# FireMines/zk_stark_project

Measured on NVIDIA B200. Metric: stark_proofs_per_sec, higher is better.
Workload: dtype u128 mod p (f128 field, 4x u32 limbs), u32 BLAKE3

## Files before the change

### zk_stark_project_b200/csrc/kernels.cuh

```cuda
#pragma once
#include "f128.cuh"
#include "blake3.cuh"
#include "coin.cuh"

namespace zkb {

struct PowTab {
    const fe* lo;
    const fe* hi;
    uint32_t l1;
};
__device__ __forceinline__ fe powtab(const PowTab& t, uint32_t e) {
    fe a = fe_ldg(t.lo + (e & ((1u << t.l1) - 1u)));
    fe b = fe_ldg(t.hi + (e >> t.l1));
    return fe_mul(a, b);
}

struct LdeMat {
    fe* data;
    uint32_t log_n, log_beta, w, log_p;
    uint32_t log_shard, bw, bw_magic, view, q_self;
    uint64_t blk_stride;
    uint32_t k0, log_kc;
};
// ... 14 lines not shown
    const uint32_t panel = (uint32_t)(gid >> lslots);
    const uint32_t slot = m.view == 0 ? s : ((m.q_self << m.log_p) + s);
    const uint32_t k = m.k0 + (panel >> lt), t_low = panel & ((1u << lt) - 1u);
    const uint32_t i = t_low + (slot << lt);
    return {k, i, compact ? (((uint64_t)i << m.log_kc) + (k - m.k0)) : (((uint64_t)i << m.log_beta) + k - leaf0)};
}
__device__ __forceinline__ size_t lde_col_off(const LdeMat& m, uint32_t j) {
    const uint32_t blk = (j * m.bw_magic) >> 16;
    return (size_t)blk * m.blk_stride + ((size_t)(j - blk * m.bw) << m.log_p);
}
__device__ __forceinline__ size_t lde_addr(const LdeMat& m, uint32_t k, uint32_t i, uint32_t j) {
    return lde_row_base(m, k, i) + lde_col_off(m, j);
}

__global__ void k_transpose_cols(const fe* __restrict__ in, fe* __restrict__ out, uint32_t n, uint32_t wc, uint32_t out_stride) {
    __shared__ uint4 tile[32][33];
    const uint32_t i0 = blockIdx.x * 32, j0 = blockIdx.y * 32;
    for (uint32_t jj = threadIdx.y; jj < 32; jj += blockDim.y) {
        uint32_t j = j0 + jj, i = i0 + threadIdx.x;
        if (j < wc && i < n) {
            const fe v = fe_canon(fe_load(in + (size_t)j * n + i), 0);
            tile[jj][threadIdx.x] = make_uint4(v.x[0], v.x[1], v.x[2], v.x[3]);
        }
    }
    __syncthreads();
    for (uint32_t ii = threadIdx.y; ii < 32; ii += blockDim.y) {
        uint32_t i = i0 + ii, j = j0 + threadIdx.x;
        if (j < wc && i < n) reinterpret_cast<uint4*>(out)[(size_t)i * out_stride + j] = tile[threadIdx.x][ii];
    }
}

struct NttPass {
    const fe* in;
    fe* out;
    uint32_t log_n, a, b;
    uint32_t w_in, w_out;
    uint32_t col0_in, col0_out, ncols, cj;
    uint32_t n_cosets, coset0;
    uint64_t in_coset_stride, out_coset_stride;
    uint32_t coset;
    uint32_t inverse;
    uint32_t log_tab;
    uint32_t log_lde;
    uint32_t out_panel;
    uint32_t log_shard;
    uint32_t panel_k0, log_kc;
    uint32_t do_scale;
    fe scale;
    PowTab roots;
    const fe* pow3;
    const fe* tw_tab;
    uint32_t tw_four;
    uint32_t tile0;
};

__device__ __forceinline__ uint32_t bitrev(uint32_t v, uint32_t bits) { return bits == 0 ? 0u : (__brev(v) >> (32 - bits)); }

__device__ __forceinline__ fe tw_mul(const fe& x, const fe& w) { return fe_mul(x, w); }
__device__ __forceinline__ fe tw_mul(const fe& x, const fe4& w) { return fe_mul_pre4(x, w); }

template <int RHO, int NC, class TW>
__device__ __forceinline__ void ntt_unit(fe* __restrict__ col, const uint32_t rs, const uint32_t cstride, const TW* __restrict__ tw,
                                         const uint32_t base, const uint32_t lam0) {
    constexpr int R = 1 << RHO;
    fe x[NC][R];
    const uint32_t step = rs << lam0;
    fe* p = col + base * rs;
#pragma unroll
    for (int c = 0; c < NC; c++)
#pragma unroll
        for (int d = 0; d < R; d++) x[c][d] = p[d * step + c * cstride];
    const uint32_t base_low = base & ((1u << lam0) - 1u);
#pragma unroll
    for (int s = 0; s < RHO; s++) {
        const TW* twl = tw + ((1u << (lam0 + s)) - 1u) + base_low;
#pragma unroll
        for (int t = 0; t < (1 << s); t++) {
            const TW w = twl[(uint32_t)t << lam0];
#pragma unroll
            for (int g = 0; g < (R >> (s + 1)); g++) {
                const int d0 = g * (2 << s) + t, d1 = d0 + (1 << s);
#pragma unroll
                for (int c = 0; c < NC; c++) {
                    const fe u = x[c][d0];
                    const fe v = tw_mul(x[c][d1], w);
                    x[c][d0] = fe_add(u, v);
                    x[c][d1] = fe_sub(u, v);
                }
            }
        }
    }
#pragma unroll
    for (int c = 0; c < NC; c++)
#pragma unroll
        for (int d = 0; d < R; d++) p[d * step + c * cstride] = x[c][d];
}

__device__ __forceinline__ fe ntt_twiddle(const NttPass& p, uint32_t k, uint32_t t_low, uint32_t q) {
    const uint32_t logS = p.b - p.a;
    const uint32_t tab_mask = (1u << p.log_tab) - 1u;
    const uint32_t lam = 32 - __clz(q + 1);
    const uint32_t th = q + 1 - (1u << (lam - 1));
    const uint32_t l = p.a + lam;
    (void)logS;
    uint32_t e = (t_low << (p.log_tab - l)) + (th << (p.log_tab - lam));
    if (p.coset) e += (k << (p.log_n - l)) << (p.log_tab - p.log_lde);
// ... 73 lines not shown
        asm volatile("cp.async.commit_group;" ::: "memory");
    } else {
        const fe* t = p.tw_tab ? p.tw_tab + ((size_t)(k << p.a) + t_low) * (S - 1u) : nullptr;
        for (uint32_t q = threadIdx.x; q + 1 < S; q += blockDim.x) {
            const fe w = t ? fe_ldg(t + q) : ntt_twiddle(p, k, t_low, q);
            if (PRE) tw[q] = fe4_from(w); else tw1[q] = w;
        }
    }
    const uint32_t c_base = ct << log_cj;
    const uint32_t log_bd = 31 - __clz(blockDim.x), log_dv = log_bd - log_cj;
    const uint32_t jj_t = threadIdx.x & (cj - 1u), v_t = threadIdx.x >> log_cj, dv = 1u << log_dv;
    const uint32_t nrow = v_t < S ? ((S - 1u - v_t) >> log_dv) + 1u : 0u;
    const bool col_ok = c_base + jj_t < p.ncols;
    {
        const size_t vstride = ((size_t)p.w_in << (p.log_n - p.b)) << p.a;
        const fe* src = p.in + (size_t)kk * p.in_coset_stride + (((size_t)u0 << p.a) + t_low) * p.w_in + p.col0_in + c_base + jj_t +
                        (size_t)v_t * vstride;
        const size_t dstride = (size_t)dv * vstride;
        char* smc = reinterpret_cast<char*>(sm + jj_t);
        const uint32_t brs = (32u - logS) & 31u;
        const uint32_t rs16 = rs * 16u;
        uint32_t vs = v_t << brs;
        const uint32_t dvs = dv << brs;
        if (col_ok) {
#pragma unroll 4
            for (uint32_t i = 0; i < nrow; i++, vs += dvs, src += dstride) *reinterpret_cast<fe*>(smc + __brev(vs) * rs16) = fe_load(src);
        } else {
            for (uint32_t i = 0; i < nrow; i++, vs += dvs) *reinterpret_cast<fe*>(smc + __brev(vs) * rs16) = fe_zero();
        }
    }
    if (PRE) asm volatile("cp.async.wait_all;" ::: "memory");
    __syncthreads();
    if (PRE) { if (cj >= 16) ntt_rounds<2>(sm, tw, rs, log_cj, logS); else ntt_rounds<1>(sm, tw, rs, log_cj, logS); }
    else ntt_rounds<1>(sm, tw1, rs, log_cj, logS);
    if (p.out_panel) {
        const size_t panel = ((size_t)(k - p.panel_k0) << p.a) + t_low;
        const uint32_t lp = logS - p.log_shard;
        const size_t np = (size_t)1 << (p.log_kc + p.a);
        const size_t chunk_stride = (np * p.w_out) << lp;
        const bool wide = S >= blockDim.x;
        const uint32_t th0 = wide ? threadIdx.x : (threadIdx.x & (S - 1u)), dth = wide ? blockDim.x : S;
        const uint32_t jj0 = wide ? 0u : (threadIdx.x >> logS), log_djj = wide ? 0u : log_bd - logS, djj = 1u << log_djj;
        const uint32_t jend = min(cj, p.ncols - c_base);
        const uint32_t ncol = jj0 < jend ? ((jend - 1u - jj0) >> log_djj) + 1u : 0u;
        const size_t cstep = (size_t)djj << lp;
        fe* colp = p.out + ((panel * p.w_out + p.col0_out + c_base + jj0) << lp);
#pragma unroll 1
        for (uint32_t th = th0; th < S; th += dth) {
            fe* d = colp + (size_t)(th >> lp) * chunk_stride + (th & ((1u << lp) - 1u));
            const fe* s = sm + th * rs + jj0;
#pragma unroll 4
            for (uint32_t j = 0; j < ncol; j++, d += cstep, s += djj) fe_store(d, *s);
        }
    } else {
        const size_t tstride = (size_t)p.w_out << p.a;
        fe* dst = p.out + (size_t)kk * p.out_coset_stride + (((size_t)u0 << p.b) + t_low) * p.w_out + p.col0_out + c_base + jj_t +
                  (size_t)v_t * tstride;
        const size_t dstride = (size_t)dv * tstride;
        const fe* s = sm + v_t * rs + jj_t;
        const uint32_t sstep = dv * rs;
        if (col_ok) {
            if (p.do_scale) {
                for (uint32_t i = 0; i < nrow; i++, dst += dstride, s += sstep) fe_store(dst, fe_mul(*s, p.scale));
            } else {
#pragma unroll 4
                for (uint32_t i = 0; i < nrow; i++, dst += dstride, s += sstep) fe_store(dst, *s);
            }
        }
    }
}

__global__ void k_scale_pow(fe* x, uint64_t n, PowTab base, fe scale, uint64_t keep, uint32_t* __restrict__ bad_degree) {
    uint64_t m = (uint64_t)blockIdx.x * blockDim.x + threadIdx.x;
    if (m >= n) return;
    const fe v = fe_load(x + m);
    if (m >= keep) { if (!fe_is_zero(v)) atomicOr(bad_degree, 1u); return; }
    fe f = fe_mul(powtab(base, (uint32_t)m), scale);
    fe_store(x + m, fe_mul(v, f));
}

__global__ void __launch_bounds__(128) k_hash_lde_rows(const LdeMat m, uint32_t* __restrict__ leaves, uint64_t leaf0, uint32_t compact) {
    const uint64_t gid = (uint64_t)blockIdx.x * blockDim.x + threadIdx.x;
    const uint32_t lpf = lde_full_log_p(m), lt = m.log_n - lpf;
    const uint32_t log_rows = m.log_kc + lt + (m.view == 0 ? lpf : m.log_p);
    if (gid >> log_rows) return;
    const LdeLeaf L = lde_leaf(m, gid, leaf0, compact);
    uint32_t d[8];
    b3_hash_elems(m.data + lde_row_base(m, L.k, L.i), (size_t)1 << m.log_p, m.w, d, m.bw, m.bw_magic, m.blk_stride);
    uint4* o = reinterpret_cast<uint4*>(leaves + L.r * 8);
    o[0] = make_uint4(d[0], d[1], d[2], d[3]);
    o[1] = make_uint4(d[4], d[5], d[6], d[7]);
}
__global__ void __launch_bounds__(128) k_hash_lde_rows_split(const LdeMat m, uint32_t* __restrict__ leaves, uint64_t leaf0, uint32_t compact) {
    const uint64_t t = (uint64_t)blockIdx.x * blockDim.x + threadIdx.x;
    const uint32_t c = (uint32_t)t & 3u;
    const uint32_t lpf = lde_full_log_p(m), lt = m.log_n - lpf;
    const uint32_t log_rows = m.log_kc + lt + (m.view == 0 ? lpf : m.log_p);
    const bool live = ((t >> 2) >> log_rows) == 0;
    const LdeLeaf L = lde_leaf(m, live ? (t >> 2) : 0, leaf0, compact);
    const uint32_t nchunks = (m.w + 63u) / 64u;
    uint32_t cv[8], nb[8];
    if (c < nchunks) b3_chunk_cv_elems(m.data + lde_row_base(m, L.k, L.i), (size_t)1 << m.log_p, m.w, c, cv, m.bw, m.bw_magic, m.blk_stride);
    else {
#pragma unroll
        for (int q = 0; q < 8; q++) cv[q] = 0;
    }
// ... 287 lines not shown
    fe s = fe_zero();
    if (j < w) for (uint32_t c = gy; c < nchunks; c += 32) s = fe_add(s, fe_load(part + (size_t)c * w + j));
    red[gy][jx] = make_uint4(s.x[0], s.x[1], s.x[2], s.x[3]);
    __syncthreads();
    for (uint32_t h = 16; h > 0; h >>= 1) {
        if (gy < h) {
            uint4 o = red[gy + h][jx];
            fe t; t.x[0] = o.x; t.x[1] = o.y; t.x[2] = o.z; t.x[3] = o.w;
            s = fe_add(s, t);
            red[gy][jx] = make_uint4(s.x[0], s.x[1], s.x[2], s.x[3]);
        }
        __syncthreads();
    }
    if (gy == 0 && j < w) fe_store(out + j, s);
}
__global__ void __launch_bounds__(256) k_poly_eval_partial(const fe* __restrict__ coef, uint32_t n, uint32_t Q, const DevTs* __restrict__ ts,
                                                           fe* __restrict__ part) {
    const fe z = ts->z, zQ = ts->zR;
    const uint32_t t = blockIdx.x * blockDim.x + threadIdx.x;
    const uint32_t nt = (n + Q - 1) / Q;
    if (t >= nt) return;
    const fe* c = coef + (size_t)blockIdx.y * n;
    const uint32_t m0 = t * Q, m1 = min(n, m0 + Q);
    fe a = fe_zero();
    for (uint32_t m = m1; m-- > m0;) a = fe_add(fe_mul(a, z), fe_load(c + m));
    fe_store(part + (size_t)t * gridDim.y + blockIdx.y, fe_mul(a, fe_pow_u64(zQ, t)));
}

__global__ void __launch_bounds__(256) k_deep_combine(const fe* __restrict__ polys, uint32_t n, uint32_t w,
                                                      const fe* __restrict__ gamma, const fe* __restrict__ hcoef, uint32_t c,
                                                      const fe* __restrict__ gamma_h, fe* __restrict__ ab) {
    const uint32_t row = (blockIdx.x * blockDim.x + threadIdx.x) / ZKB_ROW_LANES, sub = threadIdx.x & (ZKB_ROW_LANES - 1);
    if (row >= n) return;
    acc288 acc; acc288_zero(acc);
    const fe* pr = polys + (size_t)row * w;
    uint32_t j = sub;
    for (; j + 3 * ZKB_ROW_LANES < w; j += 4 * ZKB_ROW_LANES) {
        const fe v0 = fe_load(pr + j), v1 = fe_load(pr + j + ZKB_ROW_LANES), v2 = fe_load(pr + j + 2 * ZKB_ROW_LANES), v3 = fe_load(pr + j + 3 * ZKB_ROW_LANES);
        acc288_mad(acc, v0, fe_ldg(gamma + j));
        acc288_mad(acc, v1, fe_ldg(gamma + j + ZKB_ROW_LANES));
        acc288_mad(acc, v2, fe_ldg(gamma + j + 2 * ZKB_ROW_LANES));
        acc288_mad(acc, v3, fe_ldg(gamma + j + 3 * ZKB_ROW_LANES));
    }
    for (; j < w; j += ZKB_ROW_LANES) acc288_mad(acc, fe_load(pr + j), fe_ldg(gamma + j));
    acc288 hacc; acc288_zero(hacc);
    for (uint32_t i = sub; i < c; i += ZKB_ROW_LANES) acc288_mad(hacc, fe_load(hcoef + (size_t)i * n + row), fe_ldg(gamma_h + i));
    const fe s = fe_group_sum(acc288_reduce(acc));
    const fe b = c ? fe_group_sum(acc288_reduce(hacc)) : fe_zero();
    if (sub == 0) {
        fe_store(ab + (size_t)row * 2, s);
        fe_store(ab + (size_t)row * 2 + 1, fe_add(s, b));
    }
}
#define ZKB_DEEP_RPT 8
template <int RPT>
__global__ void __launch_bounds__(128) k_deep_eval(const LdeMat m, const DevTs* __restrict__ ts, PowTab roots, uint32_t log_tab,
                                                   fe* __restrict__ out, uint32_t compact) {
    const fe z = ts->z, zg = ts->zg, abz = ts->abz, azg = ts->azg;
    const uint32_t log_N = m.log_n + m.log_beta;
    const uint64_t N = (uint64_t)1 << (m.log_n + m.log_kc);
    const uint64_t nthreads = N / RPT;
    const uint64_t tid = (uint64_t)blockIdx.x * blockDim.x + threadIdx.x;
    if (tid >= nthreads) return;
    const uint32_t lt = m.log_n - m.log_p;
    fe d[2 * RPT], pre[2 * RPT], n1[RPT], n2[RPT];
    uint32_t rr[RPT];
    fe acc = fe_one();
#pragma unroll
    for (int s = 0; s < RPT; s++) {
        const uint64_t gid = tid + (uint64_t)s * nthreads;
        const uint32_t slot = (uint32_t)gid & ((1u << m.log_p) - 1u);
        const uint32_t panel = (uint32_t)(gid >> m.log_p);
        const uint32_t k = m.k0 + (panel >> lt), t_low = panel & ((1u << lt) - 1u);
        const uint32_t i = t_low + (slot << lt);
        const uint32_t r = (i << m.log_beta) + k;
        rr[s] = compact ? ((i << m.log_kc) + (k - m.k0)) : r;
        const fe* row = m.data + (((size_t)panel * 2) << m.log_p) + slot;
        fe a = fe_load(row), ab = fe_load(row + ((size_t)1 << m.log_p));
        fe x = powtab(roots, r << (log_tab - log_N));
        { fe x2 = fe_add(x, x); x = fe_add(x2, x); }
        n1[s] = fe_sub(ab, abz);
        n2[s] = fe_sub(a, azg);
        d[2 * s] = fe_sub(x, z);
        d[2 * s + 1] = fe_sub(x, zg);
        pre[2 * s] = acc; acc = fe_mul(acc, d[2 * s]);
        pre[2 * s + 1] = acc; acc = fe_mul(acc, d[2 * s + 1]);
    }
    fe ia = fe_inv(acc);
#pragma unroll
    for (int s = RPT - 1; s >= 0; s--) {
        fe i2 = fe_mul(ia, pre[2 * s + 1]); ia = fe_mul(ia, d[2 * s + 1]);
        fe i1 = fe_mul(ia, pre[2 * s]); ia = fe_mul(ia, d[2 * s]);
        fe_store(out + rr[s], fe_add(fe_mul(n1[s], i1), fe_mul(n2[s], i2)));
    }
}

struct FriFoldParams {
    const fe* in; fe* out;
    uint32_t log_m;
    const fe* alpha;
    fe inv3, inv_f;
    fe wf_inv[8];
    PowTab roots; uint32_t log_tab;
};
template <int LOG_F>
__global__ void __launch_bounds__(128) k_fri_fold(const FriFoldParams p) {
    constexpr int F = 1 << LOG_F;
    static_assert(LOG_F >= 1 && F / 2 <= (int)(sizeof(p.wf_inv) / sizeof(fe)), "folding factor out of range");
    const uint64_t rows = ((uint64_t)1 << p.log_m) >> LOG_F;
    const uint64_t i = (uint64_t)blockIdx.x * blockDim.x + threadIdx.x;
    if (i >= rows) return;
    fe v[F];
#pragma unroll
    for (int j = 0; j < F; j++) {
        const int br = (int)(__brev((unsigned)j) >> (32 - LOG_F));
        v[br] = fe_load(p.in + i + (uint64_t)j * rows);
    }
#pragma unroll
    for (int lam = 1; lam <= LOG_F; lam++) {
        const int half = 1 << (lam - 1);
#pragma unroll
        for (int q = 0; q < F / 2; q++) {
            const int th = q & (half - 1);
            const int p0 = ((q >> (lam - 1)) << lam) + th;
            fe u = v[p0];
            fe t = th == 0 ? v[p0 + half] : fe_mul(v[p0 + half], p.wf_inv[th * ((F / 2) >> (lam - 1))]);
            v[p0] = fe_add(u, t);
            v[p0 + half] = fe_sub(u, t);
        }
    }
    const uint32_t tab_mask = (1u << p.log_tab) - 1u;
    const uint32_t e = (0u - ((uint32_t)i << (p.log_tab - p.log_m))) & tab_mask;
    const fe t = fe_mul(fe_mul(fe_ldg(p.alpha), p.inv3), powtab(p.roots, e));
    fe acc = v[F - 1];
#pragma unroll
    for (int kq = F - 2; kq >= 0; kq--) acc = fe_add(fe_mul(acc, t), v[kq]);
    fe_store(p.out + i, fe_mul(acc, p.inv_f));
}

__global__ void k_gather_lde_rows(const LdeMat m, const uint32_t* __restrict__ pos, uint32_t npos, fe* __restrict__ out) {
    const uint32_t idx = blockIdx.x * blockDim.x + threadIdx.x;
    if (idx >= npos * m.w) return;
    const uint32_t q = idx / m.w, j = idx - q * m.w;
    const uint32_t r = __ldg(pos + q);
    const uint32_t k = r & ((1u << m.log_beta) - 1u), i = r >> m.log_beta;
    if (k - m.k0 >= (1u << m.log_kc)) { fe_store(out + idx, fe_zero()); return; }
// ... 171 lines not shown
```

### zk_stark_project_b200/csrc/zkb200.cu

```cuda
#include <cuda_runtime.h>
#include <dlfcn.h>
#include <sys/random.h>
#include <nccl.h>
#include <atomic>
#include <chrono>
#include <cstdio>
#include <cstdlib>
#include <functional>
#include <map>
#include <thread>
#include <tuple>
#include <memory>
#include "kernels.cuh"
#include "host.hpp"

namespace zkb {

struct CudaError : std::runtime_error { using std::runtime_error::runtime_error; };
struct StateError : std::runtime_error { using std::runtime_error::runtime_error; };

#define CK(call)                                                                                              \
    do {                                                                                                      \
        cudaError_t e_ = (call);                                                                              \
        if (e_ != cudaSuccess)                                                                                \
// ... 36 lines not shown
        return it == map.end() ? nullptr : &it->second;
    }
    bool full(size_t size) const { return bytes + size > budget && !map.empty(); }
    DevBuf& insert(const Key& k, size_t size, cudaStream_t stream) {
        if (full(size)) {
            CK(cudaStreamSynchronize(stream));
            release();
        }
        DevBuf& b = map[k];
        try { b.ensure(size); } catch (...) { map.erase(k); throw; }
        bytes += size;
        return b;
    }
    void release() {
        for (auto& kv : map) kv.second.release();
        map.clear();
        bytes = 0;
    }
};

static inline fe to_fe(const HF& h) {
    fe r;
    r.x[0] = (uint32_t)h.v; r.x[1] = (uint32_t)(h.v >> 32); r.x[2] = (uint32_t)(h.v >> 64); r.x[3] = (uint32_t)(h.v >> 96);
    return r;
}

enum Stage { ST_IDLE = 0, ST_BEGUN, ST_TRACE, ST_EVAL, ST_COMP, ST_OOD, ST_DEEP, ST_FRI_DONE, ST_QUERY };

}

using namespace zkb;

struct zkb_ctx {
    int device = 0;
    cudaStream_t stream = nullptr;
    std::string err;
    uint64_t launches = 0;
    int sm_count = 148;

    AirSpec air;
    Stage stage = ST_IDLE;
    uint32_t log_n = 0, log_beta = 0, log_N = 0, log_ce = 0, c = 0;
    uint32_t log_tab = 0;
    HostCoin coin;
    ProofParts parts;
    zkb_transcript ts;
    zkb_stage_times times;
    HF z, zg, deep_alpha;
    std::vector<HF> ood_cur, ood_next, ood_h;
    uint32_t fri_layer = 0, fri_layers = 0;
    bool fri_committed = false;
    std::vector<uint32_t> positions;

    DevBuf d_trace, d_bufA, d_bufB, d_tmp1, d_tmp2, d_lde, d_tree, d_small, d_comp_evals, d_comp_lde, d_comp_tree, d_ab, d_ab_lde,
        d_deep, d_roots_lo, d_roots_hi, d_inv3_lo, d_inv3_hi, d_pow3, d_aux, d_gather, d_user_trace, d_flags;
    std::vector<DevBuf> d_fri_evals, d_fri_tree;
    fe* d_polys = nullptr;
    uint32_t lde_log_p = 0, comp_log_p = 0, ab_log_p = 0;
    uint32_t tab_log_built = 0, pow3_for_log_n = 0, pow3_for_beta = 0;
    PowTab roots{}, inv3tab{};
    uint32_t inv3_l1 = 0;
    enum { TS_LDE, TS_XCHG, TS_LEAF, TS_MERKLE, TS_CONSTR, TS_COMP, TS_OOD, TS_DEEP, TS_FRI, TS_GRIND, TS_QUERY, TS_TOTAL, TS_COUNT };
    cudaEvent_t tev[TS_COUNT][2];
    bool trec[TS_COUNT] = {};
    bool times_valid = true;
    uint8_t* h_stage = nullptr;
    size_t h_stage_cap = 0, h_stage_used = 0;
    std::vector<HF> per_cache, per_cache_params;
    uint64_t per_cache_n = 0, per_cache_ce = 0;
    cudaEvent_t ev_group[17];
    cudaStream_t copy_stream = nullptr;
    bool owns_stream = false;
    cudaStream_t xchg_stream = nullptr;
    bool ev_ok = false;

    ncclComm_t comm = nullptr;
    int mg_rank = 0, mg_world = 1;
    uint32_t log_g = 0;
    bool mg_active = false;
    DevBuf d_bnd_coef, d_bnd_lde;

    struct FsTree { size_t o_rows, o_paths; uint32_t width, depth; };
    struct FsLayout { size_t o_ood = 0, o_rem = 0, host_bytes = 0, o_coef = 0, o_gamma = 0, o_scr = 0, total = 0; uint32_t rem_cap = 0; std::vector<FsTree> trees; } fs;
    DevBuf d_fs, d_in, d_rem_coef;
    ShapeCache<std::string> pack_cache{(size_t)64 << 20};
    ShapeCache<std::vector<uint64_t>> div_cache{(size_t)2 << 30};
    struct GraphEntry { cudaGraphExec_t exec = nullptr; uint64_t epoch = 0; uint32_t seen = 0; uint64_t launches = 0; };
    std::map<std::string, GraphEntry> graphs;
    bool capturing = false;
    uint8_t* h_out = nullptr;
    size_t h_out_cap = 0;
    cudaEvent_t ev_done = nullptr;
    DevTs* dts() const { return d_fs.as<DevTs>(); }
    fe* fs_fe(size_t off) const { return reinterpret_cast<fe*>(d_fs.as<uint8_t>() + off); }
    const fe* d_aval() const { return d_in.as<fe>(); }
    const fe* d_params() const { return d_in.as<fe>() + air.assertions.size(); }
    DevBuf d_lde_rows, d_mg_a, d_mg_b;
    DevBuf d_cap;

    void count() { launches++; }
    static uint32_t magic16(uint32_t d) { return (65536u + d - 1) / d; }
    LdeMat std_mat(fe* data, uint32_t w, uint32_t log_p) const { return LdeMat{data, log_n, log_beta, w, log_p, 0, w, magic16(w), 0, 0, 0, 0, log_beta}; }
    bool mg_coset() const { return mg_active && (uint32_t)mg_world <= air.blowup; }
    uint32_t mg_log_kc() const { return log_beta - log_g; }
    LdeMat coset_mat(fe* data, uint32_t w, uint32_t log_p) const {
        LdeMat m = std_mat(data, w, log_p);
        if (mg_coset()) { m.log_kc = mg_log_kc(); m.k0 = (uint32_t)mg_rank << m.log_kc; }
        return m;
    }
    LdeMat lde_mat() const {
        if (!mg_active) return std_mat(d_lde.as<fe>(), air.w, lde_log_p);
        const uint32_t wl = air.w / (uint32_t)mg_world;
        return LdeMat{d_lde.as<fe>(), log_n, log_beta, wl, lde_log_p - log_g, log_g, wl, magic16(wl), 0, (uint32_t)mg_rank, 0, 0, log_beta};
    }
    LdeMat lde_rows_mat() const {
        const uint32_t wl = air.w / (uint32_t)mg_world, lp = lde_log_p - log_g;
        const uint64_t np = (uint64_t)1 << (log_beta + log_n - lde_log_p);
        return LdeMat{d_lde_rows.as<fe>(), log_n, log_beta, air.w, lp, log_g, wl, magic16(wl), 1, (uint32_t)mg_rank, (np * wl) << lp, 0, log_beta};
    }
    LdeMat comp_mat() const { return coset_mat(d_comp_lde.as<fe>(), c, comp_log_p); }
    LdeMat ab_mat() const { return coset_mat(d_ab_lde.as<fe>(), 2, ab_log_p); }

    void init(int dev, void* strm) {
        int ndev = 0;
        cudaError_t e = cudaGetDeviceCount(&ndev);
        if (e != cudaSuccess || ndev == 0) throw CudaError(std::string("no CUDA device available: ") + cudaGetErrorString(e));
        if (dev < 0 || dev >= ndev) throw InvalidArg("device index out of range");
        device = dev;
        CK(cudaSetDevice(device));
        stream = (cudaStream_t)strm;
        cudaDeviceProp prop;
        CK(cudaGetDeviceProperties(&prop, device));
        sm_count = prop.multiProcessorCount;
        CK(cudaFuncSetAttribute(k_ntt_pass<true>, cudaFuncAttributeMaxDynamicSharedMemorySize, 200 * 1024));
        CK(cudaFuncSetAttribute(k_ntt_pass<false>, cudaFuncAttributeMaxDynamicSharedMemorySize, 200 * 1024));
        for (auto& pr : tev) for (auto& x : pr) CK(cudaEventCreate(&x));
        h_stage_cap = (size_t)8 << 20;
        CK(cudaHostAlloc((void**)&h_stage, h_stage_cap, cudaHostAllocDefault));
        for (auto& x : ev_group) CK(cudaEventCreateWithFlags(&x, cudaEventDisableTiming));
        CK(cudaEventCreateWithFlags(&ev_done, cudaEventBlockingSync | cudaEventDisableTiming));
        CK(cudaStreamCreateWithFlags(&copy_stream, cudaStreamNonBlocking));
        {
            int lo = 0, hi = 0;
            CK(cudaDeviceGetStreamPriorityRange(&lo, &hi));
            CK(cudaStreamCreateWithPriority(&xchg_stream, cudaStreamNonBlocking, hi));
        }
        ev_ok = true;
        memset(&times, 0, sizeof(times));
    }
    void destroy() {
        cudaSetDevice(device);
        cudaStreamSynchronize(stream);
        for (DevBuf* b : {&d_trace, &d_bufA, &d_bufB, &d_tmp1, &d_tmp2, &d_lde, &d_tree, &d_small, &d_comp_evals, &d_comp_lde, &d_comp_tree,
                          &d_ab, &d_ab_lde, &d_deep, &d_roots_lo, &d_roots_hi, &d_inv3_lo, &d_inv3_hi, &d_pow3, &d_aux, &d_gather, &d_user_trace, &d_flags,
                          &d_lde_rows, &d_mg_a, &d_mg_b, &d_cap, &d_bnd_coef, &d_bnd_lde, &d_fs, &d_in, &d_rem_coef})
            b->release();
        if (comm) { g_nccl.CommDestroy(comm); comm = nullptr; }
        for (auto& b : d_fri_evals) b.release();
        for (auto& b : d_fri_tree) b.release();
        tw_cache.release();
        pack_cache.release();
        div_cache.release();
        for (auto& kv : graphs) if (kv.second.exec) cudaGraphExecDestroy(kv.second.exec);
        if (ev_ok) { for (auto& pr : tev) for (auto& x : pr) cudaEventDestroy(x); for (auto& x : ev_group) cudaEventDestroy(x); cudaStreamDestroy(copy_stream); cudaStreamDestroy(xchg_stream); }
        if (h_stage) cudaFreeHost(h_stage);
        if (h_out) cudaFreeHost(h_out);
        if (ev_done) cudaEventDestroy(ev_done);
        if (owns_stream && stream) { cudaStreamDestroy(stream); stream = nullptr; }
    }

    void h2d(void* dst, const void* src, size_t bytes) { CK(cudaMemcpyAsync(dst, src, bytes, cudaMemcpyHostToDevice, stream)); }
    void h2d_small(void* dst, const void* src, size_t bytes) {
        if (bytes == 0) return;
        const size_t need = (bytes + 255) & ~(size_t)255;
        if (h_stage_used + need > h_stage_cap) {
            CK(cudaMemcpyAsync(dst, src, bytes, cudaMemcpyHostToDevice, stream));
            CK(cudaStreamSynchronize(stream));
            return;
        }
        memcpy(h_stage + h_stage_used, src, bytes);
        CK(cudaMemcpyAsync(dst, h_stage + h_stage_used, bytes, cudaMemcpyHostToDevice, stream));
        h_stage_used += need;
    }
    void t_begin(int st) { if (!capturing) CK(cudaEventRecord(tev[st][0], stream)); }
    void t_end(int st) { if (!capturing) { CK(cudaEventRecord(tev[st][1], stream)); trec[st] = true; times_valid = false; } }
    void collect_times() {
        if (times_valid) return;
        CK(cudaSetDevice(device));
        CK(cudaStreamSynchronize(stream));
        float* slot[TS_COUNT] = {&times.lde, &times.interpolate, &times.leaf_hash, &times.merkle, &times.constraints, &times.composition,
                                 &times.ood, &times.deep, &times.fri, &times.grind, &times.queries, &times.total};
        for (int st = 0; st < TS_COUNT; st++) if (trec[st]) CK(cudaEventElapsedTime(slot[st], tev[st][0], tev[st][1]));
        times_valid = true;
    }
    void d2h(void* dst, const void* src, size_t bytes) {
        CK(cudaMemcpyAsync(dst, src, bytes, cudaMemcpyDeviceToHost, stream));
        CK(cudaStreamSynchronize(stream));
    }
    void check_launch() { CK(cudaGetLastError()); count(); }

    static void build_powtab(HF base, uint32_t log_size, std::vector<HF>& lo, std::vector<HF>& hi, uint32_t& l1) {
        l1 = (log_size + 1) / 2;
        uint32_t l2 = log_size - l1;
        lo.resize((size_t)1 << l1); hi.resize((size_t)1 << l2);
        HF x = HF::raw(1);
        for (auto& v : lo) { v = x; x = x * base; }
        HF step = x;
// ... 31 lines not shown
    static std::vector<uint32_t> plan_layers(uint32_t log_len, uint32_t cj) {
        uint32_t maxlog = pre_twiddles(cj) ? (cj >= 16 ? 8 : 9) : 12 - log2u(cj);
        uint32_t passes = (log_len + maxlog - 1) / maxlog;
        if (passes == 0) passes = 1;
        std::vector<uint32_t> b;
        uint32_t done = 0;
        for (uint32_t q = 0; q < passes; q++) { uint32_t take = (log_len - done + (passes - q) - 1) / (passes - q); done += take; b.push_back(done); }
        return b;
    }
    ShapeCache<std::tuple<uint32_t, uint32_t, uint32_t, uint32_t, uint32_t, uint32_t, uint32_t>> tw_cache{(size_t)768 << 20};
    void twiddle_table(NttPass& p, uint32_t all_cosets) {
        const uint32_t S = 1u << (p.b - p.a);
        const uint64_t entries = ((uint64_t)all_cosets << p.a) * (S - 1u);
        const bool pre = pre_twiddles(p.cj);
        const uint64_t cap = (uint64_t)(pre ? 64 : 192) << 20;
        p.tw_tab = nullptr; p.tw_four = 0;
        static const bool log_tables = getenv("ZKB_HOST_PROFILE") != nullptr;
        if (S < 2 || entries * 16 > cap) {
            if (log_tables && S >= 2)
                fprintf(stderr, "[zkb twiddles] log_n %u layers [%u, %u) coset %u inverse %u cj %u: no table (%.2f MiB plain), generated\n", p.log_n,
                        p.a, p.b, p.coset, p.inverse, p.cj, entries * 16 / 1048576.0);
            return;
        }
        const uint32_t four = pre && entries * 64 <= cap ? 1u : 0u;
        const uint64_t bytes = entries * (four ? 64 : 16);
        const auto key = std::make_tuple(p.log_n, p.a, p.b, p.coset, p.inverse, p.coset ? p.log_lde : 0u, four);
        DevBuf* tab = tw_cache.find(key);
        if (!tab) {
            if (log_tables && tw_cache.full(bytes)) fprintf(stderr, "[zkb twiddles] cache of %.2f MiB over budget: cleared\n", tw_cache.bytes / 1048576.0);
            tab = &tw_cache.insert(key, bytes, stream);
            if (log_tables)
                fprintf(stderr, "[zkb twiddles] log_n %u layers [%u, %u) coset %u inverse %u cj %u: %s table %.2f MiB, cache %.2f MiB\n", p.log_n, p.a,
                        p.b, p.coset, p.inverse, p.cj, four ? "four-copy" : "plain", bytes / 1048576.0, tw_cache.bytes / 1048576.0);
            NttPass q = p;
            q.n_cosets = all_cosets; q.coset0 = 0; q.tw_four = four;
            k_build_twiddles<<<(unsigned)((entries + 255) / 256), 256, 0, stream>>>(q, tab->as<fe>());
            check_launch();
        }
        p.tw_tab = tab->as<fe>(); p.tw_four = four;
    }
    void launch_pass(NttPass p) {
        const uint32_t S = 1u << (p.b - p.a);
        const uint32_t rs = p.cj + (p.cj > 1 ? 1 : 0);
        const bool pre = pre_twiddles(p.cj);
        const size_t smem = ((size_t)S * rs + (pre ? 4 : 1) * (size_t)S) * 16;
        const uint32_t n_ct = (p.ncols + p.cj - 1) / p.cj;
        const uint64_t tiles = (uint64_t)1 << (p.log_n - (p.b - p.a));
        if (p.n_cosets > 65535) throw InvalidArg("transform too large for one launch");
        uint32_t threads = 256;
        if (pre) {
            const uint32_t units = p.cj >= 16 ? S * p.cj / 16 : S * p.cj / 8;
            threads = std::max<uint32_t>(units, std::min<uint32_t>(S, 256));
            threads = std::min<uint32_t>(256, std::max<uint32_t>(32, threads));
        }
        for (uint64_t z0 = 0; z0 < tiles; z0 += 65535) {
            p.tile0 = (uint32_t)z0;
            const dim3 grid(n_ct, p.n_cosets, (unsigned)std::min<uint64_t>(65535, tiles - z0));
            if (pre) k_ntt_pass<true><<<grid, threads, smem, stream>>>(p);
            else k_ntt_pass<false><<<grid, threads, smem, stream>>>(p);
            check_launch();
        }
    }
    struct Xform {
        const fe* in; uint32_t w_in, col0_in;
        fe* out; uint32_t w_out, col0_out;
        uint32_t ncols, log_len;
        bool inverse, coset_lde;
        uint32_t log_lde;
        bool scale; HF scale_by;
        uint32_t log_shard = 0;
        uint32_t coset_lo = 0, coset_cnt = 0;
        uint32_t batch_cosets = 0;
        std::function<void(uint32_t, uint32_t)> after_batch;
        uint32_t cj = 0;
    };
    uint32_t run_xform(const Xform& x, DevBuf& s1, DevBuf& s2) {
        const uint32_t cj = x.cj ? x.cj : pick_cj(x.ncols);
        std::vector<uint32_t> bnd = plan_layers(x.log_len, cj);
        const uint32_t passes = (uint32_t)bnd.size();
        const uint64_t len = (uint64_t)1 << x.log_len;
        const uint32_t all_cosets = x.coset_lde ? (1u << (x.log_lde - x.log_len)) : 1;
        const uint32_t n_cosets = (x.coset_lde && x.coset_cnt) ? x.coset_cnt : all_cosets;
        uint32_t batch = x.batch_cosets ? std::min(x.batch_cosets, n_cosets) : n_cosets;
        if (passes > 1) {
            const uint64_t per = len * x.ncols * 16;
            uint64_t budget = (uint64_t)6 << 30;
            batch = (uint32_t)std::max<uint64_t>(1, std::min<uint64_t>(batch, budget / std::max<uint64_t>(per, 1)));
            s1.ensure(per * batch);
            if (passes > 2) s2.ensure(per * batch);
        }
        for (uint32_t k0 = 0; k0 < n_cosets; k0 += batch) {
            const uint32_t nk = std::min(batch, n_cosets - k0);
            uint32_t a = 0;
            const fe* src = x.in; uint32_t w_src = x.w_in, c0_src = x.col0_in; uint64_t src_stride = 0;
            for (uint32_t q = 0; q < passes; q++) {
                NttPass p{};
                const bool last = (q + 1 == passes);
                p.in = src; p.w_in = w_src; p.col0_in = c0_src; p.in_coset_stride = src_stride;
                p.log_n = x.log_len; p.a = a; p.b = bnd[q];
                p.ncols = x.ncols; p.cj = cj; p.n_cosets = nk; p.coset0 = x.coset_lo + k0;
                p.panel_k0 = x.coset_lo; p.log_kc = log2u(n_cosets);
                p.coset = x.coset_lde ? 1 : 0; p.inverse = x.inverse ? 1 : 0;
                p.log_tab = log_tab; p.log_lde = x.coset_lde ? x.log_lde : 0;
                p.roots = roots; p.pow3 = d_pow3.as<fe>();
                twiddle_table(p, all_cosets);
                if (last) {
                    p.out = x.out; p.w_out = x.w_out; p.col0_out = x.col0_out;
                    p.out_panel = x.coset_lde ? 1 : 0;
                    p.log_shard = x.coset_lde ? x.log_shard : 0;
                    if (p.log_shard > p.b - p.a) throw InvalidArg("trace too short to shard its LDE panels across this many GPUs");
                    p.out_coset_stride = 0;
                    p.do_scale = x.scale ? 1 : 0; p.scale = to_fe(x.scale_by);
                } else {
                    fe* dst = (q % 2 == 0) ? s1.as<fe>() : s2.as<fe>();
                    p.out = dst; p.w_out = x.ncols; p.col0_out = 0; p.out_coset_stride = len * x.ncols;
                    src = dst; w_src = x.ncols; c0_src = 0; src_stride = len * x.ncols;
                }
                launch_pass(p);
                a = bnd[q];
            }
            if (x.after_batch) x.after_batch(x.coset_lo + k0, nk);
        }
        return bnd.back() - (passes > 1 ? bnd[passes - 2] : 0);
    }

    void build_merkle(uint32_t* heap, uint64_t n_leaves) {
        uint64_t lvl = n_leaves / 2;
        for (; lvl > 512; lvl >>= 1) {
            k_merkle_level<<<(unsigned)((lvl + 255) / 256), 256, 0, stream>>>(heap + 2 * lvl * 8, heap + lvl * 8, lvl);
            check_launch();
        }
        k_merkle_top<<<1, 512, 0, stream>>>(heap, (uint32_t)lvl);
        check_launch();
    }

    void begin(const zkb_air_desc* desc) {
        CK(cudaSetDevice(device));
        air = AirSpec::from_desc(desc);
        log_n = log2u(air.n); log_beta = log2u(air.blowup); log_N = log_n + log_beta;
        log_ce = log2u(air.ce_blowup()); c = air.num_comp_cols();
        if ((1u << log_ce) > air.blowup) throw InvalidArg("constraint evaluation blowup exceeds the LDE blowup");
        {
            std::set<uint64_t> steps;
            for (auto& a : air.assertions) steps.insert(a.step);
            if (steps.size() > ZKB_MAX_GROUPS) throw InvalidArg("too many distinct assertion steps (boundary groups)");
        }
        ensure_tables();
        parts = ProofParts();
        memset(&ts, 0, sizeof(ts));
        ts.comp_degree_ok = 1;
        memset(&times, 0, sizeof(times));
        for (auto& r : trec) r = false;
        times_valid = true;
        h_stage_used = 0;
        coin.init(air.coin_seed());
        fri_layers = air.num_fri_layers();
        if (fri_layers > ZKB_MAX_FRI_LAYERS) throw InvalidArg("too many FRI layers");
        fri_layer = 0; fri_committed = false;
        positions.clear();
        mg_active = false;
        {
// ... 439 lines not shown
                                                                   nch == 1 ? nxt_out : sm + o_pzg);
        check_launch();
        if (nch > 1) { col_sum(sm + o_pz, nch, wl, cur_out); col_sum(sm + o_pzg, nch, wl, nxt_out); }
        {
            dim3 grid((nt + 255) / 256, c);
            k_poly_eval_partial<<<grid, 256, 0, stream>>>(d_bufA.as<fe>(), (uint32_t)n, Q, dts(), nt == 1 ? frame + 2 * (size_t)w : sm + o_hp);
            check_launch();
            if (nt > 1) col_sum(sm + o_hp, nt, c, frame + 2 * (size_t)w);
        }
        if (mg_active) {
            NK(g_nccl.AllGather(sm + o_loc, sm + o_ga, 2 * (size_t)wl * 16, ncclUint8, comm, stream));
            for (uint32_t h = 0; h < 2; h++)
                CK(cudaMemcpy2DAsync(frame + (size_t)h * w, (size_t)wl * 16, sm + o_ga + (size_t)h * wl, 2 * (size_t)wl * 16, (size_t)wl * 16, (size_t)mg_world,
                                     cudaMemcpyDeviceToDevice, stream));
        }
        t_end(TS_OOD);
        stage = ST_OOD;
    }
    void ood_fetch() {
        const uint32_t w = air.w;
        std::vector<HF> host(2 * (size_t)w + c);
        d2h(host.data(), fs_fe(fs.o_ood), host.size() * 16);
        ood_cur.assign(host.begin(), host.begin() + w);
        ood_next.assign(host.begin() + w, host.begin() + 2 * (size_t)w);
        ood_h.assign(host.begin() + 2 * (size_t)w, host.end());
    }
    void ood_eval(const HF& z_) {
        if (stage != ST_COMP) throw StateError("zkb_ood_eval: constraint commitment is missing");
        z = z_; zg = z * HF::root_of_unity(log_n);
        fs_after_constraint_root(nullptr, &z_);
        ood_eval_dev();
        ood_fetch();
    }

    void deep_compose_dev() {
        if (stage != ST_OOD) throw StateError("zkb_deep_compose: OOD frame is missing");
        t_begin(TS_DEEP);
        const uint64_t n = air.n, N = air.lde_size(); const uint32_t w = air.w;
        const fe* gamma = fs_fe(fs.o_gamma);
        d_ab.ensure(n * 2 * 16);
        if (!mg_active) {
            k_deep_combine<<<(unsigned)((n * ZKB_ROW_LANES + 255) / 256), 256, 0, stream>>>(d_polys, (uint32_t)n, w, gamma, d_bufA.as<fe>(), c, gamma + w, d_ab.as<fe>());
            check_launch();
        } else {
            const uint32_t wl = w / (uint32_t)mg_world;
            d_mg_a.ensure(n * 2 * 16);
            k_deep_combine<<<(unsigned)((n * ZKB_ROW_LANES + 255) / 256), 256, 0, stream>>>(d_polys, (uint32_t)n, wl, gamma + (size_t)mg_rank * wl, d_bufA.as<fe>(), 0,
                                                                              gamma + w, d_mg_a.as<fe>());
            check_launch();
            mg_field_allreduce(d_mg_a.as<fe>(), 2 * n, d_ab.as<fe>());
            k_deep_add_h<<<(unsigned)((n + 255) / 256), 256, 0, stream>>>(d_ab.as<fe>(), (uint32_t)n, d_bufA.as<fe>(), c, gamma + w);
            check_launch();
        }
        d_ab_lde.ensure(N * 2 * 16);
        d_deep.ensure(N * 16);
        if (!mg_coset()) {
            Xform x{d_ab.as<fe>(), 2, 0, d_ab_lde.as<fe>(), 2, 0, 2, log_n, false, true, log_N, false, HF()};
            ab_log_p = run_xform(x, d_tmp1, d_tmp2);
            if (N <= 8192) k_deep_eval<1><<<(unsigned)((N + 127) / 128), 128, 0, stream>>>(ab_mat(), dts(), roots, log_tab, d_deep.as<fe>(), 0);
            else k_deep_eval<ZKB_DEEP_RPT><<<(unsigned)((N / ZKB_DEEP_RPT + 127) / 128), 128, 0, stream>>>(ab_mat(), dts(), roots, log_tab, d_deep.as<fe>(), 0);
            check_launch();
        } else {
            const uint32_t kc = 1u << mg_log_kc();
            const uint64_t Nloc = n * kc;
            Xform x{d_ab.as<fe>(), 2, 0, d_ab_lde.as<fe>(), 2, 0, 2, log_n, false, true, log_N, false, HF()};
            x.coset_lo = (uint32_t)mg_rank * kc; x.coset_cnt = kc;
            ab_log_p = run_xform(x, d_tmp1, d_tmp2);
            d_mg_a.ensure(Nloc * 16); d_mg_b.ensure(N * 16);
            const uint64_t threads = Nloc / ZKB_DEEP_RPT;
            k_deep_eval<ZKB_DEEP_RPT><<<(unsigned)((threads + 127) / 128), 128, 0, stream>>>(ab_mat(), dts(), roots, log_tab, d_mg_a.as<fe>(), 1);
            check_launch();
            NK(g_nccl.AllGather(d_mg_a.p, d_mg_b.p, Nloc * 16, ncclUint8, comm, stream));
            k_permute_coset_items<<<(unsigned)((N + 255) / 256), 256, 0, stream>>>(d_mg_b.as<uint32_t>(), d_deep.as<uint32_t>(), log_n, log_beta,
                                                                               mg_log_kc(), 4);
            check_launch();
        }
        t_end(TS_DEEP);
        if (d_fri_evals.size() < fri_layers + 1) { d_fri_evals.resize(fri_layers + 1); d_fri_tree.resize(fri_layers + 1); }
        fri_layer = 0; fri_committed = false;
        stage = ST_DEEP;
    }
    void deep_compose(const HF& alpha) {
        if (stage != ST_OOD) throw StateError("zkb_deep_compose: OOD frame is missing");
        deep_alpha = alpha;
        fs_after_ood(false, &alpha);
        deep_compose_dev();
    }

    const fe* fri_cur_evals() const { return fri_layer == 0 ? d_deep.as<fe>() : d_fri_evals[fri_layer].as<fe>(); }
    uint64_t fri_domain(uint32_t layer) const { return air.lde_size() >> (air.log_folding() * layer); }
    uint64_t fri_rows(uint32_t layer) const { return fri_domain(layer) >> air.log_folding(); }
    void fri_commit_layer_dev() {
        if (stage != ST_DEEP || fri_layer >= fri_layers || fri_committed) throw StateError("zkb_fri_commit_layer: out of order");
        const uint64_t rows = fri_rows(fri_layer);
        DevBuf& tree = d_fri_tree[fri_layer];
        tree.ensure(2 * rows * 32);
        k_hash_strided_rows<<<(unsigned)((rows + 127) / 128), 128, 0, stream>>>(fri_cur_evals(), rows, air.folding, tree.as<uint32_t>() + rows * 8);
        check_launch();
        build_merkle(tree.as<uint32_t>(), rows);
        fri_committed = true;
    }
    static constexpr uint32_t TS_FRI_SLOTS = sizeof(zkb_transcript::fri_roots) / sizeof(zkb_transcript::fri_roots[0]);
    void fri_commit_layer(uint8_t root_out[32]) {
        fri_commit_layer_dev();
        uint8_t spare[32];
        take_root(d_fri_tree[fri_layer].as<uint32_t>() + 8, fri_layer < TS_FRI_SLOTS ? ts.fri_roots[fri_layer] : spare, root_out);
    }
    void fri_fold_dev() {
        if (stage != ST_DEEP || !fri_committed) throw StateError("zkb_fri_fold: commit the layer first");
        const uint64_t rows = fri_rows(fri_layer);
        DevBuf& nxt = d_fri_evals[fri_layer + 1];
        nxt.ensure(rows * sizeof(fe));
        FriFoldParams p{};
        p.in = fri_cur_evals(); p.out = nxt.as<fe>(); p.log_m = log2u(fri_domain(fri_layer));
        p.alpha = &dts()->fri_alpha[fri_layer]; p.inv3 = to_fe(HF::from_u64(3).inv()); p.inv_f = to_fe(HF::from_u64(air.folding).inv());
        HF wi = HF::root_of_unity(air.log_folding()).inv(), x = HF::raw(1);
        for (uint32_t q = 0; q < air.folding / 2; q++) { p.wf_inv[q] = to_fe(x); x = x * wi; }
        p.roots = roots; p.log_tab = log_tab;
        const dim3 grid((unsigned)((rows + 127) / 128)), block(128);
        switch (air.log_folding()) {
            case 1: k_fri_fold<1><<<grid, block, 0, stream>>>(p); break;
            case 2: k_fri_fold<2><<<grid, block, 0, stream>>>(p); break;
            case 3: k_fri_fold<3><<<grid, block, 0, stream>>>(p); break;
            case 4: k_fri_fold<4><<<grid, block, 0, stream>>>(p); break;
// ... 677 lines not shown
```

Before: 82.09.

## Compute DEEP quotient in coefficient space via scan before a single-column LDE

```diff
diff --git a/zk_stark_project_b200/csrc/kernels.cuh b/zk_stark_project_b200/csrc/kernels.cuh
--- a/zk_stark_project_b200/csrc/kernels.cuh
+++ b/zk_stark_project_b200/csrc/kernels.cuh
@@ -90,6 +90,7 @@
     const fe* tw_tab;
     uint32_t tw_four;
     uint32_t tile0;
+    uint32_t out_natural;
 };
 
 __device__ __forceinline__ uint32_t bitrev(uint32_t v, uint32_t bits) { return bits == 0 ? 0u : (__brev(v) >> (32 - bits)); }
@@ -269,6 +270,9 @@
 #pragma unroll 4
             for (uint32_t j = 0; j < ncol; j++, d += cstep, s += djj) fe_store(d, *s);
         }
+    } else if (!PRE && p.out_natural) {
+        fe* d = p.out + ((size_t)t_low << p.log_kc) + (k - p.panel_k0);
+        for (uint32_t th = threadIdx.x; th < S; th += blockDim.x) fe_store(d + ((size_t)th << (p.a + p.log_kc)), sm[th * rs]);
     } else {
         const size_t tstride = (size_t)p.w_out << p.a;
         fe* dst = p.out + (size_t)kk * p.out_coset_stride + (((size_t)u0 << p.b) + t_low) * p.w_out + p.col0_out + c_base + jj_t +
@@ -662,46 +666,85 @@
         fe_store(ab + (size_t)row * 2 + 1, fe_add(s, b));
     }
 }
-#define ZKB_DEEP_RPT 8
-template <int RPT>
-__global__ void __launch_bounds__(128) k_deep_eval(const LdeMat m, const DevTs* __restrict__ ts, PowTab roots, uint32_t log_tab,
-                                                   fe* __restrict__ out, uint32_t compact) {
-    const fe z = ts->z, zg = ts->zg, abz = ts->abz, azg = ts->azg;
-    const uint32_t log_N = m.log_n + m.log_beta;
-    const uint64_t N = (uint64_t)1 << (m.log_n + m.log_kc);
-    const uint64_t nthreads = N / RPT;
-    const uint64_t tid = (uint64_t)blockIdx.x * blockDim.x + threadIdx.x;
-    if (tid >= nthreads) return;
-    const uint32_t lt = m.log_n - m.log_p;
-    fe d[2 * RPT], pre[2 * RPT], n1[RPT], n2[RPT];
-    uint32_t rr[RPT];
-    fe acc = fe_one();
-#pragma unroll
-    for (int s = 0; s < RPT; s++) {
-        const uint64_t gid = tid + (uint64_t)s * nthreads;
-        const uint32_t slot = (uint32_t)gid & ((1u << m.log_p) - 1u);
-        const uint32_t panel = (uint32_t)(gid >> m.log_p);
-        const uint32_t k = m.k0 + (panel >> lt), t_low = panel & ((1u << lt) - 1u);
-        const uint32_t i = t_low + (slot << lt);
-        const uint32_t r = (i << m.log_beta) + k;
-        rr[s] = compact ? ((i << m.log_kc) + (k - m.k0)) : r;
-        const fe* row = m.data + (((size_t)panel * 2) << m.log_p) + slot;
-        fe a = fe_load(row), ab = fe_load(row + ((size_t)1 << m.log_p));
-        fe x = powtab(roots, r << (log_tab - log_N));
-        { fe x2 = fe_add(x, x); x = fe_add(x2, x); }
-        n1[s] = fe_sub(ab, abz);
-        n2[s] = fe_sub(a, azg);
-        d[2 * s] = fe_sub(x, z);
-        d[2 * s + 1] = fe_sub(x, zg);
-        pre[2 * s] = acc; acc = fe_mul(acc, d[2 * s]);
-        pre[2 * s + 1] = acc; acc = fe_mul(acc, d[2 * s + 1]);
-    }
-    fe ia = fe_inv(acc);
-#pragma unroll
-    for (int s = RPT - 1; s >= 0; s--) {
-        fe i2 = fe_mul(ia, pre[2 * s + 1]); ia = fe_mul(ia, d[2 * s + 1]);
-        fe i1 = fe_mul(ia, pre[2 * s]); ia = fe_mul(ia, d[2 * s]);
-        fe_store(out + rr[s], fe_add(fe_mul(n1[s], i1), fe_mul(n2[s], i2)));
+#define ZKB_QUOT_L 16
+#define ZKB_QUOT_THREADS 256
+__device__ __forceinline__ void quot_scan(uint4 (*sh)[ZKB_QUOT_THREADS], fe v[4]) {
+    const uint32_t t = threadIdx.x;
+#pragma unroll 1
+    for (uint32_t d = 1; d < ZKB_QUOT_THREADS; d <<= 1) {
+#pragma unroll
+        for (int q = 0; q < 4; q++) fe_store(reinterpret_cast<fe*>(&sh[q][t]), v[q]);
+        __syncthreads();
+        if (t + d < ZKB_QUOT_THREADS) {
+#pragma unroll
+            for (int h = 0; h < 2; h++) {
+                const fe s = fe_load(reinterpret_cast<const fe*>(&sh[2 * h][t + d])), m = fe_load(reinterpret_cast<const fe*>(&sh[2 * h + 1][t + d]));
+                v[2 * h] = fe_add(v[2 * h], fe_mul(v[2 * h + 1], s));
+                v[2 * h + 1] = fe_mul(v[2 * h + 1], m);
+            }
+        }
+        __syncthreads();
+    }
+#pragma unroll
+    for (int q = 0; q < 4; q++) fe_store(reinterpret_cast<fe*>(&sh[q][t]), v[q]);
+    __syncthreads();
+}
+template <bool AGG>
+__global__ void __launch_bounds__(ZKB_QUOT_THREADS) k_deep_quotient(const fe* __restrict__ ab, uint32_t n, const DevTs* __restrict__ ts,
+                                                                     fe* __restrict__ agg, fe* __restrict__ out) {
+    __shared__ uint4 sh[4][ZKB_QUOT_THREADS];
+    const fe c[2] = {ts->z, ts->zg};
+    const uint32_t t = threadIdx.x, b = blockIdx.x;
+    const uint32_t m0 = (b * ZKB_QUOT_THREADS + t) * ZKB_QUOT_L;
+    auto coef = [&](uint32_t m, int h) { return m < n ? fe_load(ab + 2 * (size_t)m + 1 - h) : fe_zero(); };
+    fe v[4];
+#pragma unroll
+    for (int h = 0; h < 2; h++) {
+        fe s = fe_zero();
+#pragma unroll
+        for (int j = ZKB_QUOT_L - 1; j >= 0; j--) s = fe_add(fe_mul(s, c[h]), coef(m0 + j, h));
+        v[2 * h] = s;
+        v[2 * h + 1] = fe_sqr_n(c[h], 4);
+    }
+    static_assert(ZKB_QUOT_L == 16, "v[2h+1] = c^ZKB_QUOT_L");
+    quot_scan(sh, v);
+    if (AGG) {
+        if (t == 0) { fe_store(agg + 2 * (size_t)b, v[0]); fe_store(agg + 2 * (size_t)b + 1, v[2]); }
+        return;
+    }
+    fe up[4], mb[2];
+    const bool last = t + 1 == ZKB_QUOT_THREADS;
+#pragma unroll
+    for (int q = 0; q < 4; q++) up[q] = last ? (q & 1 ? fe_one() : fe_zero()) : fe_load(reinterpret_cast<const fe*>(&sh[q][t + 1]));
+    mb[0] = fe_load(reinterpret_cast<const fe*>(&sh[1][0]));
+    mb[1] = fe_load(reinterpret_cast<const fe*>(&sh[3][0]));
+    __syncthreads();
+    fe cb[2] = {fe_zero(), fe_zero()};
+    const uint32_t above = gridDim.x - 1u - b;
+#pragma unroll 1
+    for (uint32_t ch = (above + ZKB_QUOT_THREADS - 1u) / ZKB_QUOT_THREADS; ch-- > 0;) {
+        const uint32_t k = ch * ZKB_QUOT_THREADS + t;
+        fe a[4];
+#pragma unroll
+        for (int h = 0; h < 2; h++) {
+            a[2 * h] = k < above ? fe_load(agg + 2 * (size_t)(b + 1 + k) + h) : fe_zero();
+            a[2 * h + 1] = k < above ? mb[h] : fe_one();
+        }
+        quot_scan(sh, a);
+#pragma unroll
+        for (int h = 0; h < 2; h++)
+            cb[h] = fe_add(fe_load(reinterpret_cast<const fe*>(&sh[2 * h][0])), fe_mul(fe_load(reinterpret_cast<const fe*>(&sh[2 * h + 1][0])), cb[h]));
+        __syncthreads();
+    }
+    fe q[2];
+#pragma unroll
+    for (int h = 0; h < 2; h++) q[h] = fe_add(up[2 * h], fe_mul(up[2 * h + 1], cb[h]));
+#pragma unroll
+    for (int j = ZKB_QUOT_L - 1; j >= 0; j--) {
+        const uint32_t m = m0 + j;
+        if (m < n) fe_store(out + m, fe_add(q[0], q[1]));
+#pragma unroll
+        for (int h = 0; h < 2; h++) q[h] = fe_add(coef(m, h), fe_mul(c[h], q[h]));
     }
 }
 
diff --git a/zk_stark_project_b200/csrc/zkb200.cu b/zk_stark_project_b200/csrc/zkb200.cu
--- a/zk_stark_project_b200/csrc/zkb200.cu
+++ b/zk_stark_project_b200/csrc/zkb200.cu
@@ -112,11 +112,11 @@
     bool fri_committed = false;
     std::vector<uint32_t> positions;
 
-    DevBuf d_trace, d_bufA, d_bufB, d_tmp1, d_tmp2, d_lde, d_tree, d_small, d_comp_evals, d_comp_lde, d_comp_tree, d_ab, d_ab_lde,
+    DevBuf d_trace, d_bufA, d_bufB, d_tmp1, d_tmp2, d_lde, d_tree, d_small, d_comp_evals, d_comp_lde, d_comp_tree, d_ab, d_deep_poly,
         d_deep, d_roots_lo, d_roots_hi, d_inv3_lo, d_inv3_hi, d_pow3, d_aux, d_gather, d_user_trace, d_flags;
     std::vector<DevBuf> d_fri_evals, d_fri_tree;
     fe* d_polys = nullptr;
-    uint32_t lde_log_p = 0, comp_log_p = 0, ab_log_p = 0;
+    uint32_t lde_log_p = 0, comp_log_p = 0;
     uint32_t tab_log_built = 0, pow3_for_log_n = 0, pow3_for_beta = 0;
     PowTab roots{}, inv3tab{};
     uint32_t inv3_l1 = 0;
@@ -179,7 +179,6 @@
         return LdeMat{d_lde_rows.as<fe>(), log_n, log_beta, air.w, lp, log_g, wl, magic16(wl), 1, (uint32_t)mg_rank, (np * wl) << lp, 0, log_beta};
     }
     LdeMat comp_mat() const { return coset_mat(d_comp_lde.as<fe>(), c, comp_log_p); }
-    LdeMat ab_mat() const { return coset_mat(d_ab_lde.as<fe>(), 2, ab_log_p); }
 
     void init(int dev, void* strm) {
         int ndev = 0;
@@ -212,7 +211,7 @@
         cudaSetDevice(device);
         cudaStreamSynchronize(stream);
         for (DevBuf* b : {&d_trace, &d_bufA, &d_bufB, &d_tmp1, &d_tmp2, &d_lde, &d_tree, &d_small, &d_comp_evals, &d_comp_lde, &d_comp_tree,
-                          &d_ab, &d_ab_lde, &d_deep, &d_roots_lo, &d_roots_hi, &d_inv3_lo, &d_inv3_hi, &d_pow3, &d_aux, &d_gather, &d_user_trace, &d_flags,
+                          &d_ab, &d_deep_poly, &d_deep, &d_roots_lo, &d_roots_hi, &d_inv3_lo, &d_inv3_hi, &d_pow3, &d_aux, &d_gather, &d_user_trace, &d_flags,
                           &d_lde_rows, &d_mg_a, &d_mg_b, &d_cap, &d_bnd_coef, &d_bnd_lde, &d_fs, &d_in, &d_rem_coef})
             b->release();
         if (comm) { g_nccl.CommDestroy(comm); comm = nullptr; }
@@ -350,6 +349,8 @@
             const uint32_t units = p.cj >= 16 ? S * p.cj / 16 : S * p.cj / 8;
             threads = std::max<uint32_t>(units, std::min<uint32_t>(S, 256));
             threads = std::min<uint32_t>(256, std::max<uint32_t>(32, threads));
+        } else {
+            threads = std::min<uint32_t>(256, std::max<uint32_t>(32, S * p.cj / 8));
         }
         for (uint64_t z0 = 0; z0 < tiles; z0 += 65535) {
             p.tile0 = (uint32_t)z0;
@@ -370,10 +371,12 @@
         uint32_t coset_lo = 0, coset_cnt = 0;
         uint32_t batch_cosets = 0;
         std::function<void(uint32_t, uint32_t)> after_batch;
+        bool natural = false;
         uint32_t cj = 0;
     };
     uint32_t run_xform(const Xform& x, DevBuf& s1, DevBuf& s2) {
         const uint32_t cj = x.cj ? x.cj : pick_cj(x.ncols);
+        if (x.natural && (!x.coset_lde || x.ncols != 1 || x.log_shard)) throw InvalidArg("natural LDE order is for one unsharded column");
         std::vector<uint32_t> bnd = plan_layers(x.log_len, cj);
         const uint32_t passes = (uint32_t)bnd.size();
         const uint64_t len = (uint64_t)1 << x.log_len;
@@ -404,7 +407,8 @@
                 twiddle_table(p, all_cosets);
                 if (last) {
                     p.out = x.out; p.w_out = x.w_out; p.col0_out = x.col0_out;
-                    p.out_panel = x.coset_lde ? 1 : 0;
+                    p.out_panel = x.coset_lde && !x.natural ? 1 : 0;
+                    p.out_natural = x.natural ? 1 : 0;
                     p.log_shard = x.coset_lde ? x.log_shard : 0;
                     if (p.log_shard > p.b - p.a) throw InvalidArg("trace too short to shard its LDE panels across this many GPUs");
                     p.out_coset_stride = 0;
@@ -950,24 +954,27 @@
             k_deep_add_h<<<(unsigned)((n + 255) / 256), 256, 0, stream>>>(d_ab.as<fe>(), (uint32_t)n, d_bufA.as<fe>(), c, gamma + w);
             check_launch();
         }
-        d_ab_lde.ensure(N * 2 * 16);
+        const uint32_t nb = (uint32_t)((n + ZKB_QUOT_THREADS * ZKB_QUOT_L - 1) / (ZKB_QUOT_THREADS * ZKB_QUOT_L));
+        d_deep_poly.ensure((n + 2 * (uint64_t)nb) * 16);
+        fe* agg = d_deep_poly.as<fe>() + n;
+        if (nb > 1) {
+            k_deep_quotient<true><<<nb, ZKB_QUOT_THREADS, 0, stream>>>(d_ab.as<fe>(), (uint32_t)n, dts(), agg, nullptr);
+            check_launch();
+        }
+        k_deep_quotient<false><<<nb, ZKB_QUOT_THREADS, 0, stream>>>(d_ab.as<fe>(), (uint32_t)n, dts(), agg, d_deep_poly.as<fe>());
+        check_launch();
         d_deep.ensure(N * 16);
+        Xform x{d_deep_poly.as<fe>(), 1, 0, d_deep.as<fe>(), 1, 0, 1, log_n, false, true, log_N, false, HF()};
+        x.natural = true;
         if (!mg_coset()) {
-            Xform x{d_ab.as<fe>(), 2, 0, d_ab_lde.as<fe>(), 2, 0, 2, log_n, false, true, log_N, false, HF()};
-            ab_log_p = run_xform(x, d_tmp1, d_tmp2);
-            if (N <= 8192) k_deep_eval<1><<<(unsigned)((N + 127) / 128), 128, 0, stream>>>(ab_mat(), dts(), roots, log_tab, d_deep.as<fe>(), 0);
-            else k_deep_eval<ZKB_DEEP_RPT><<<(unsigned)((N / ZKB_DEEP_RPT + 127) / 128), 128, 0, stream>>>(ab_mat(), dts(), roots, log_tab, d_deep.as<fe>(), 0);
-            check_launch();
+            run_xform(x, d_tmp1, d_tmp2);
         } else {
             const uint32_t kc = 1u << mg_log_kc();
             const uint64_t Nloc = n * kc;
-            Xform x{d_ab.as<fe>(), 2, 0, d_ab_lde.as<fe>(), 2, 0, 2, log_n, false, true, log_N, false, HF()};
+            d_mg_a.ensure(Nloc * 16); d_mg_b.ensure(N * 16);
+            x.out = d_mg_a.as<fe>();
             x.coset_lo = (uint32_t)mg_rank * kc; x.coset_cnt = kc;
-            ab_log_p = run_xform(x, d_tmp1, d_tmp2);
-            d_mg_a.ensure(Nloc * 16); d_mg_b.ensure(N * 16);
-            const uint64_t threads = Nloc / ZKB_DEEP_RPT;
-            k_deep_eval<ZKB_DEEP_RPT><<<(unsigned)((threads + 127) / 128), 128, 0, stream>>>(ab_mat(), dts(), roots, log_tab, d_mg_a.as<fe>(), 1);
-            check_launch();
+            run_xform(x, d_tmp1, d_tmp2);
             NK(g_nccl.AllGather(d_mg_a.p, d_mg_b.p, Nloc * 16, ncclUint8, comm, stream));
             k_permute_coset_items<<<(unsigned)((N + 255) / 256), 256, 0, stream>>>(d_mg_b.as<uint32_t>(), d_deep.as<uint32_t>(), log_n, log_beta,
                                                                                mg_log_kc(), 4);
```

After: 84.27, median of 6. 1.03x the previous value.
